# davipatti/abdpymc

Hardware: AMD Instinct MI355X
Metric: logp+grad evals/sec (higher is better)
Workload: dtype f64; 1 GPU; synthetic 10000 ind x 200 gaps, fp64, 4 chains/GPU; n_inds=10000, n_gaps=200, storage=f64, chains_per_gpu=4, total_chains=4, parallelism=chains sharded 4/GPU x 1

## Files before the change

### abdpymc_amd/csrc/abd_dense.hpp

```cpp
#pragma once

#include <cstddef>

#include "abd_device.hpp"
#include "abd_planes.hpp"
#include "abd_terms.hpp"

typedef uint32_t abd_u32x4 __attribute__((ext_vector_type(4)));
typedef uint32_t abd_u32x2 __attribute__((ext_vector_type(2)));
template <typename R>
__device__ __forceinline__ YX<R> load_yx(const __amdgpu_buffer_rsrc_t& rs, uint32_t voff, uint32_t soff);
template <>
__device__ __forceinline__ YX<double> load_yx<double>(const __amdgpu_buffer_rsrc_t& rs, uint32_t voff, uint32_t soff) {
  const abd_u32x4 v = __builtin_amdgcn_raw_buffer_load_b128(rs, voff, soff, 0);
  YX<double> r;
  r.y = __hiloint2double((int)v.y, (int)v.x);
  r.x = __hiloint2double((int)v.w, (int)v.z);
  return r;
}
template <>
__device__ __forceinline__ YX<float> load_yx<float>(const __amdgpu_buffer_rsrc_t& rs, uint32_t voff, uint32_t soff) {
  const abd_u32x2 v = __builtin_amdgcn_raw_buffer_load_b64(rs, voff, soff, 0);
  YX<float> r;
  r.y = __uint_as_float(v.x);
  r.x = __uint_as_float(v.y);
  return r;
}

template <typename R, bool XC>
struct RowData;
template <typename R>
struct RowData<R, false> {
  YX<R> v;
};
template <typename R>
struct RowData<R, true> {
  R y;
  uint32_t code;
};
template <bool XC>
struct RowDesc;
template <>
struct RowDesc<false> {
  __amdgpu_buffer_rsrc_t rs;
};
template <>
struct RowDesc<true> {
  __amdgpu_buffer_rsrc_t rs_y, rs_c;
};
__device__ __forceinline__ __amdgpu_buffer_rsrc_t rsrc_at(const void* base, int64_t byte_off) {
  return __builtin_amdgcn_make_buffer_rsrc(const_cast<char*>(reinterpret_cast<const char*>(base)) + byte_off, 0, -1, 0x00020000);
}
template <typename R, bool XC, typename ARGS>
__device__ __forceinline__ RowDesc<XC> row_desc(const ARGS& a, int antigen, int lg, int g0) {
  RowDesc<XC> d;
  if constexpr (XC) {
    const int64_t cell0 = ((int64_t)lg * a.G + g0) * 64;
    d.rs_y = rsrc_at(antigen ? a.od_s : a.od_n, cell0 * (int64_t)sizeof(R));
    d.rs_c = rsrc_at(antigen ? a.xc_s : a.xc_n, cell0);
  } else {
    const int64_t cell0 = (int64_t)g0 * a.N + (int64_t)lg * 64;
    d.rs = rsrc_at(antigen ? a.yx_s : a.yx_n, cell0 * (int64_t)sizeof(YX<R>));
  }
  return d;
}
template <typename R, bool XC>
__device__ __forceinline__ RowData<R, XC> row_load(const RowDesc<XC>& d, int lane, int row, int N) {
  RowData<R, XC> r;
  if constexpr (XC) {
    const uint32_t soff = (uint32_t)row * 64u;
    if constexpr (sizeof(R) == 8) {
      const abd_u32x2 v = __builtin_amdgcn_raw_buffer_load_b64(d.rs_y, (uint32_t)lane * 8u, soff * 8u, 0);
      r.y = __hiloint2double((int)v.y, (int)v.x);
    } else {
      r.y = __uint_as_float(__builtin_amdgcn_raw_buffer_load_b32(d.rs_y, (uint32_t)lane * 4u, soff * 4u, 0));
    }
    r.code = __builtin_amdgcn_raw_buffer_load_b8(d.rs_c, (uint32_t)lane, soff, 0);
  } else {
    r.v = load_yx<R>(d.rs, (uint32_t)lane * (uint32_t)sizeof(YX<R>), (uint32_t)row * (uint32_t)N * (uint32_t)sizeof(YX<R>));
  }
  return r;
}
template <typename R, bool XC>
__device__ __forceinline__ double row_y(const RowData<R, XC>& r) {
  if constexpr (XC) return (double)r.y;
  else return (double)r.v.y;
}
template <typename R, bool XC>
__device__ __forceinline__ double row_x(const RowData<R, XC>& r, const double* dict ) {
  if constexpr (XC) return dict[r.code];
  else return (double)r.v.x;
}

__device__ __forceinline__ uint32_t word32(const uint32_t* base, uint32_t j2, int q, int N) {
  const uint32_t* row = base + ((int64_t)(q >> 1) * 2 * N + (q & 1));
  return row[j2];
}

#define ABD_EXP2_C2 0x1.ebfbe033445b4p-23
__device__ __forceinline__ void one_plus_exp2_pair(double t_n, double t_s, const double* tab , double c2v, double& A,
                                                   double& B) {
#pragma clang fp contract(off)
  const double kf_n = __builtin_rint(t_n), kf_s = __builtin_rint(t_s);
  const double f_n = t_n - kf_n, f_s = t_s - kf_s;
  int k_n, k_s;
  asm("v_cvt_i32_f64 %0, %1" : "=v"(k_n) : "v"(kf_n));
  asm("v_cvt_i32_f64 %0, %1" : "=v"(k_s) : "v"(kf_s));
  const int kc_n = min(max(k_n, ABD_EXP2_K_MIN), ABD_EXP2_K_MAX), kc_s = min(max(k_s, ABD_EXP2_K_MIN), ABD_EXP2_K_MAX);
  const double T_n = tab[kc_n & (ABD_EXP2_TAB - 1)], T_s = tab[kc_s & (ABD_EXP2_TAB - 1)];
  double p_n, p_s;
  asm("v_fma_f64 %0, %1, %2, %3" : "=v"(p_n) : "s"(0x1.c6b08d910ecbdp-35), "v"(f_n), "v"(c2v));
  asm("v_fma_f64 %0, %1, %2, %3" : "=v"(p_s) : "s"(0x1.c6b08d910ecbdp-35), "v"(f_s), "v"(c2v));
  p_n = fma(p_n, f_n, 0x1.62e42fefa39efp-11);
  p_s = fma(p_s, f_s, 0x1.62e42fefa39efp-11);
  p_n = fma(p_n, f_n, 1.0);
  p_s = fma(p_s, f_s, 1.0);
  const double Ts_n = __hiloint2double((int)abd_exp2_scaled_hi((uint32_t)__double2hiint(T_n), kc_n), __double2loint(T_n));
  const double Ts_s = __hiloint2double((int)abd_exp2_scaled_hi((uint32_t)__double2hiint(T_s), kc_s), __double2loint(T_s));
  A = fma(Ts_n, p_n, 1.0);
  B = fma(Ts_s, p_s, 1.0);
}

template <bool GRAD>
__device__ __forceinline__ void obs_pair_scaled(double t_n, double yn, double d_n, double t_s, double ys, double d_s,
                                                const double* tab, double c2v, double (&acc)[16], double& h_n, double& h_s) {
#pragma clang fp contract(off)
  double A, B;
  one_plus_exp2_pair(t_n, t_s, tab, c2v, A, B);
  const double r = rcp_newton(A * B);
  const double s_n = r * B, s_s = r * A;
  const double q_n = fma(-d_n, s_n, yn), q_s = fma(-d_s, s_s, ys);
  acc[A_N_Q2] = fma(q_n, q_n, acc[A_N_Q2]);
  acc[A_S_Q2] = fma(q_s, q_s, acc[A_S_Q2]);
  if (GRAD) {
    const double u_n = q_n * s_n, u_s = q_s * s_s;
    acc[A_N_QS] = fma(s_n, q_n, acc[A_N_QS]);
    acc[A_S_QS] = fma(s_s, q_s, acc[A_S_QS]);
    h_n = fma(-u_n, s_n, u_n);
    h_s = fma(-u_s, s_s, u_s);
    acc[A_N_H] += h_n;
    acc[A_S_H] += h_s;
    acc[A_N_HX] = fma(h_n, t_n, acc[A_N_HX]);
    acc[A_S_HX] = fma(h_s, t_s, acc[A_S_HX]);
  }
}

#ifdef ABD_STAMPS
#define ABD_STAMP(k)                                                                                  \
  do {                                                                                                \
    if (a.stamps && wave == 0 && lane == 0 && blockIdx.y == 0)                                        \
      a.stamps[(int64_t)blockIdx.x * 16 + (k)] = __builtin_amdgcn_s_memrealtime();                   \
  } while (0)
#else
#define ABD_STAMP(k)
#endif

struct DenseChain {
  double rho_n, rho_s;
  double ct_n, cp_n, ci_n, mc_n;
  double c_s, cp_s, ci_s, mc_s;
  double d_n, d_s;
};
__device__ __forceinline__ DenseChain dense_chain(const ChainPar& p) {
  DenseChain k;
  const double c_n = p.b_n * (1.4426950408889634074 * ABD_EXP2_TAB), c_s = p.b_s * (1.4426950408889634074 * ABD_EXP2_TAB);
  k.rho_n = p.rho_n;
  k.rho_s = p.rho_s;
  k.ct_n = readfirstlane_f64(c_n * p.temp_n);
  k.cp_n = readfirstlane_f64(c_n * p.perm_n);
  k.ci_n = to_vgpr(c_n * p.init_n);
  k.mc_n = readfirstlane_f64(-c_n);
  k.c_s = readfirstlane_f64(c_s);
  k.cp_s = readfirstlane_f64(c_s * p.perm_s);
  k.ci_s = to_vgpr(c_s * p.init_s);
  k.mc_s = readfirstlane_f64(-c_s);
  k.d_n = p.d_n;
  k.d_s = p.d_s;
  return k;
}

#define ABD_SW 8
template <typename R, bool XC>
struct PieceLoads {
  uint32_t seg_i, seg_v, nxt_i, nxt_v;
  RowData<R, XC> en, es, on, os;
  int wj;
};

template <typename R, bool XC, bool WORDS, typename ARGS>
__device__ __forceinline__ void piece_issue_loads(const ARGS& a, const RowDesc<XC>& rs_n, const RowDesc<XC>& rs_s,
                                                  const uint32_t* ibase, const uint32_t* vbase, const int8_t* waner, int lane, int j,
                                                  int g0, int g1, PieceLoads<R, XC>& pl) {
  const int N = a.N;
  const int q = g0 >> 5, q_end = (g1 - 1) >> 5;
  const int last = g1 - 1 - g0;
  const int re = min(g0 & 1, last), ro = min((g0 & 1) ^ 1, last);
  if (g0 & 1) {
    pl.on = row_load<R, XC>(rs_n, lane, ro, N);
    pl.os = row_load<R, XC>(rs_s, lane, ro, N);
    pl.en = row_load<R, XC>(rs_n, lane, re, N);
    pl.es = row_load<R, XC>(rs_s, lane, re, N);
  } else {
    pl.en = row_load<R, XC>(rs_n, lane, re, N);
    pl.es = row_load<R, XC>(rs_s, lane, re, N);
    pl.on = row_load<R, XC>(rs_n, lane, ro, N);
    pl.os = row_load<R, XC>(rs_s, lane, ro, N);
  }
  pl.seg_i = pl.seg_v = pl.nxt_i = pl.nxt_v = 0;
  if constexpr (WORDS) {
    const uint32_t j2 = 2u * (uint32_t)j;
    pl.seg_i = word32(ibase, j2, q, N);
    pl.seg_v = word32(vbase, j2, q, N);
    if (q < q_end) {
      pl.nxt_i = word32(ibase, j2, q + 1, N);
      pl.nxt_v = word32(vbase, j2, q + 1, N);
    }
  }
  pl.wj = waner[j];
}

__device__ __forceinline__ void state_issue_loads(const uint32_t* ibase, const uint32_t* vbase, uint32_t j2, int N, int g0,
                                                  uint32_t (&wi)[ABD_SW], uint32_t (&wv)[ABD_SW]) {
  const int qlast = (g0 - 1) >> 5;
#pragma unroll
  for (int u = 0; u < ABD_SW; ++u) {
    wi[u] = wv[u] = 0;
    if (u <= qlast) {
      wi[u] = word32(ibase, j2, u, N);
      wv[u] = word32(vbase, j2, u, N);
    }
  }
}

__device__ __forceinline__ void dense_start_state(uint32_t (&wi)[ABD_SW], uint32_t (&wv)[ABD_SW], const uint32_t* ibase,
                                                  const uint32_t* vbase, uint32_t j2, int N, int g0, const double2_t* tab_n,
                                                  const double2_t* tab_s, bool wj, double& tn, double& dn, double& ts, double& ds,
                                                  uint32_t& cfn_hi, uint32_t& cfs_hi) {
  const int qlast = (g0 - 1) >> 5;
  uint32_t any_i = 0, any_v = 0;
  int cnt = 0;
  for (int q0 = 0;; q0 += ABD_SW) {
#pragma unroll
    for (int u = 0; u < ABD_SW; ++u) {
      const int q = q0 + u;
      if (q <= qlast) {
        const int rel = g0 - q * 32;
        uint32_t mi = wi[u], mv = wv[u];
        if (rel < 32) {
          const uint32_t below = (1u << rel) - 1u;
          mi &= below;
          mv &= below;
        }
        any_i |= mi;
        any_v |= mv;
        cnt += __builtin_popcount(mi) + __builtin_popcount(mv);
        if (__builtin_amdgcn_ballot_w64((mi | mv) != 0) != 0) {
          while (mi | mv) {
            const int idx_i = mi ? rel - __builtin_ctz(mi) : 0;
            const int idx_v = mv ? rel - __builtin_ctz(mv) : 0;
            mi &= mi - 1;
            mv &= mv - 1;
            const double2_t pn = tab_n[idx_i];
            const double2_t ps = tab_s[idx_i];
            const double2_t pv = tab_s[idx_v];
            tn += pn.x;
            dn += pn.y;
            ts += ps.x;
            ds += ps.y;
            ts += pv.x;
            ds += pv.y;
          }
        }
      }
    }
    if (q0 + ABD_SW > qlast) break;
#pragma unroll
    for (int u = 0; u < ABD_SW; ++u) {
      const int q = q0 + ABD_SW + u;
      wi[u] = wv[u] = 0;
      if (q <= qlast) {
        wi[u] = word32(ibase, j2, q, N);
        wv[u] = word32(vbase, j2, q, N);
      }
    }
  }
  if (!wj) {
    ts = (double)cnt;
    ds = 0.0;
  }
  cfn_hi = any_i ? 0x3FF00000u : 0u;
  cfs_hi = (any_i | any_v) ? 0x3FF00000u : 0u;
}

template <typename R, bool GRAD, bool XC, typename ARGS>
__device__ __forceinline__ void dense_walk(const ARGS& a, const DenseChain& k, const RowDesc<XC>& rs_n,
                                           const RowDesc<XC>& rs_s, const double* dict_n, const double* dict_s,
                                           const uint32_t* ibase, const uint32_t* vbase,
                                           uint32_t j2, PieceLoads<R, XC>& pl, int lane, int g0, int g1, bool wj, double tn, double dn, double ts,
                                           double ds, uint32_t cfn_hi, uint32_t cfs_hi, const double* tab_e2, double c2v,
                                           double (&acc)[16]) {
#pragma clang fp contract(off)
  const int N = a.N;
  const double rho_n = k.rho_n, ct_n = k.ct_n, cp_n = k.cp_n, ci_n = k.ci_n, mc_n = k.mc_n;
  const double c_s = k.c_s, cp_s = k.cp_s, ci_s = k.ci_s, mc_s = k.mc_s, d_n = k.d_n, d_s = k.d_s;
  const double rho_j = wj ? k.rho_s : 1.0;
  double hd_s = 0.0;
  const uint32_t z_ei = zero_vgpr(), z_ev = zero_vgpr(), z_cn = zero_vgpr(), z_cs = zero_vgpr();
  const int last = g1 - 1 - g0;
  auto ldrow = [&](const RowDesc<XC>& rs, int g) { return row_load<R, XC>(rs, lane, min(g - g0, last), N); };
  int q = g0 >> 5;
  const int q_end = (g1 - 1) >> 5;
  uint32_t seg_i = pl.seg_i, seg_v = pl.seg_v;
  auto next_word = [&]() {
    seg_i = pl.nxt_i;
    seg_v = pl.nxt_v;
    ++q;
    if (q < q_end) {
      pl.nxt_i = word32(ibase, j2, q + 1, N);
      pl.nxt_v = word32(vbase, j2, q + 1, N);
    }
  };

  auto step = [&](int g, const RowData<R, XC>& on, const RowData<R, XC>& os) {
    const uint32_t bit = (uint32_t)g & 31u;
    const uint32_t ei_hi = (uint32_t)__builtin_amdgcn_sbfe((int)seg_i, bit, 1u) & 0x3FF00000u;
    const uint32_t ev_hi = (uint32_t)__builtin_amdgcn_sbfe((int)seg_v, bit, 1u) & 0x3FF00000u;
    const double e_i = hi_to_double(ei_hi, z_ei), e_v = hi_to_double(ev_hi, z_ev);
    cfn_hi |= ei_hi;
    cfs_hi |= ei_hi | ev_hi;
    dn = fma_s(rho_n, dn, tn);
    tn = fma_s(rho_n, tn, e_i);
    ds = fma_v(rho_j, ds, ts);
    ts = fma_v(rho_j, ts, e_i + e_v);
    const double cf_n = hi_to_double(cfn_hi, z_cn), cf_s = hi_to_double(cfs_hi, z_cs);
    const double t_n = fma(mc_n, row_x<R, XC>(on, dict_n), fma(ct_n, tn, fma(cf_n, cp_n, ci_n)));
    const double t_s = fma(mc_s, row_x<R, XC>(os, dict_s), fma(c_s, ts, fma(cf_s, cp_s, ci_s)));
    double h_n = 0.0, h_s = 0.0;
    obs_pair_scaled<GRAD>(t_n, row_y<R, XC>(on), d_n, t_s, row_y<R, XC>(os), d_s, tab_e2, c2v, acc, h_n, h_s);
    if (GRAD) {
      acc[A_N_HC] = fma(h_n, cf_n, acc[A_N_HC]);
      acc[A_N_HU] = fma(h_n, tn, acc[A_N_HU]);
      acc[A_N_HD] = fma(h_n, dn, acc[A_N_HD]);
      acc[A_S_HC] = fma(h_s, cf_s, acc[A_S_HC]);
      hd_s = fma(h_s, ds, hd_s);
    }
  };

  RowData<R, XC> en = pl.en, es = pl.es, on = pl.on, os = pl.os;
  int g = g0;
  if (g & 1) {
    step(g, on, os);
    on = ldrow(rs_n, g + 2);
    os = ldrow(rs_s, g + 2);
    ++g;
    if (g < g1 && (g & 31) == 0) next_word();
  }
  while (g + 1 < g1) {
    const int pair_end = min(((g >> 5) + 1) << 5, g1 - 1);
    for (; g < pair_end; g += 2) {
      step(g, en, es);
      en = ldrow(rs_n, g + 2);
      es = ldrow(rs_s, g + 2);
      step(g + 1, on, os);
      on = ldrow(rs_n, g + 3);
      os = ldrow(rs_s, g + 3);
    }
    if (g < g1 && (g & 31) == 0) next_word();
  }
  if (g < g1) step(g, en, es);
  acc[A_S_HD] += wj ? hd_s : 0.0;
}


typedef uint64_t abd_u64x2 __attribute__((ext_vector_type(2)));
typedef uint64_t abd_u64x4 __attribute__((ext_vector_type(4)));
static_assert(sizeof(abd_u64x2) == sizeof(PlaneGap) && sizeof(abd_u64x4) == sizeof(PlanePair), "plane layout (abd_types.hpp)");
typedef const abd_u64x2 __attribute__((address_space(4)))* plane_gap_ptr;
typedef const abd_u64x4 __attribute__((address_space(4)))* plane_pair_ptr;
__device__ __forceinline__ plane_gap_ptr plane_row(const uint64_t* planes, int lg, int G) {
  return (plane_gap_ptr)(uintptr_t)(planes + abd_plane_index(lg, 0, G, 0));
}
__device__ __forceinline__ uint32_t mask_select(uint64_t mask, uint32_t on, uint32_t off) {
  return __builtin_amdgcn_inverse_ballot_w64(mask) ? on : off;
}

template <typename R, bool GRAD, bool XC, typename ARGS>
__device__ __forceinline__ void dense_walk_planes(const ARGS& a, const DenseChain& k, const RowDesc<XC>& rs_n,
                                                  const RowDesc<XC>& rs_s, const double* dict_n, const double* dict_s,
                                                  plane_gap_ptr prow, PieceLoads<R, XC>& pl, int lane, int g0, int g1, bool wj, double tn,
                                                  double dn, double ts, double ds, uint32_t cfn_hi, uint32_t cfs_hi, ExposureSeen seen,
                                                  const double* tab_e2, double c2v, double (&acc)[16]) {
#pragma clang fp contract(off)
  const int N = a.N;
  const double rho_n = k.rho_n, ct_n = k.ct_n, mc_n = k.mc_n;
  const double c_s = k.c_s, mc_s = k.mc_s, d_n = k.d_n, d_s = k.d_s;
  const double rho_j = wj ? k.rho_s : 1.0;
  double hd_s = 0.0;
  const uint32_t z_ei = zero_vgpr(), z_ev = zero_vgpr(), z_cn = zero_vgpr(), z_cs = zero_vgpr();
  const double b1_n = fma(1.0, k.cp_n, k.ci_n), b1_s = fma(1.0, k.cp_s, k.ci_s);
  double base_n = cfn_hi ? b1_n : fma(0.0, k.cp_n, k.ci_n), base_s = cfs_hi ? b1_s : fma(0.0, k.cp_s, k.ci_s);
  const int last = g1 - 1 - g0;
  auto ldrow = [&](const RowDesc<XC>& rs, int g) { return row_load<R, XC>(rs, lane, min(g - g0, last), N); };

  auto step = [&](uint64_t m_i, uint64_t m_v, const RowData<R, XC>& on, const RowData<R, XC>& os) {
    const ExposureSeen nw = abd_exposure_new(seen, m_i, m_v);
    if ((nw.n | nw.s) != 0) {
      cfn_hi = mask_select(nw.n, 0x3FF00000u, cfn_hi);
      cfs_hi = mask_select(nw.s, 0x3FF00000u, cfs_hi);
      base_n = __hiloint2double((int)mask_select(nw.n, (uint32_t)__double2hiint(b1_n), (uint32_t)__double2hiint(base_n)),
                                (int)mask_select(nw.n, (uint32_t)__double2loint(b1_n), (uint32_t)__double2loint(base_n)));
      base_s = __hiloint2double((int)mask_select(nw.s, (uint32_t)__double2hiint(b1_s), (uint32_t)__double2hiint(base_s)),
                                (int)mask_select(nw.s, (uint32_t)__double2loint(b1_s), (uint32_t)__double2loint(base_s)));
      abd_exposure_mark(seen, m_i, m_v);
    }
    const double e_i = hi_to_double(mask_select(m_i, 0x3FF00000u, 0u), z_ei), e_v = hi_to_double(mask_select(m_v, 0x3FF00000u, 0u), z_ev);
    dn = fma_s(rho_n, dn, tn);
    tn = fma_s(rho_n, tn, e_i);
    ds = fma_v(rho_j, ds, ts);
    ts = fma_v(rho_j, ts, e_i + e_v);
    const double cf_n = hi_to_double(cfn_hi, z_cn), cf_s = hi_to_double(cfs_hi, z_cs);
    const double t_n = fma(mc_n, row_x<R, XC>(on, dict_n), fma(ct_n, tn, base_n));
    const double t_s = fma(mc_s, row_x<R, XC>(os, dict_s), fma(c_s, ts, base_s));
    double h_n = 0.0, h_s = 0.0;
    obs_pair_scaled<GRAD>(t_n, row_y<R, XC>(on), d_n, t_s, row_y<R, XC>(os), d_s, tab_e2, c2v, acc, h_n, h_s);
    if (GRAD) {
      acc[A_N_HC] = fma(h_n, cf_n, acc[A_N_HC]);
      acc[A_N_HU] = fma(h_n, tn, acc[A_N_HU]);
      acc[A_N_HD] = fma(h_n, dn, acc[A_N_HD]);
      acc[A_S_HC] = fma(h_s, cf_s, acc[A_S_HC]);
      hd_s = fma(h_s, ds, hd_s);
      asm volatile("" : "+v"(cfn_hi), "+v"(cfs_hi), "+v"(base_n), "+v"(base_s), "+v"(acc[A_N_HC]), "+v"(acc[A_S_HC]));
    } else {
      asm volatile("" : "+v"(base_n), "+v"(base_s), "+v"(acc[A_N_Q2]), "+v"(acc[A_S_Q2]));
    }
  };

  RowData<R, XC> en = pl.en, es = pl.es, on = pl.on, os = pl.os;
  int g = g0;
  abd_u64x4 cur = *(plane_pair_ptr)(prow + ((g0 + 1) & ~1));
  if (g & 1) {
    const abd_u64x2 m = prow[g];
    step(m.x, m.y, on, os);
    on = ldrow(rs_n, g + 2);
    os = ldrow(rs_s, g + 2);
    ++g;
  }
  while (g + 1 < g1) {
    const abd_u64x4 nxt = *(plane_pair_ptr)(prow + g + 2);
    __builtin_amdgcn_sched_barrier(0);
    step(cur.x, cur.y, en, es);
    en = ldrow(rs_n, g + 2);
    es = ldrow(rs_s, g + 2);
    step(cur.z, cur.w, on, os);
    on = ldrow(rs_n, g + 3);
    os = ldrow(rs_s, g + 3);
    cur = nxt;
    g += 2;
  }
  if (g < g1) step(cur.x, cur.y, en, es);
  acc[A_S_HD] += wj ? hd_s : 0.0;
}

__device__ __forceinline__ const char* train_kernarg() {
#if defined(__HIP_DEVICE_COMPILE__)
  return (const char*)__builtin_amdgcn_kernarg_segment_ptr();
#else
  return nullptr;
#endif
}
__device__ __forceinline__ const TrainPoint* train_point(const TrainArgs& T) {
  return T.use_slot >= 0 ? T.slots + T.use_slot
                         : reinterpret_cast<const TrainPoint*>(train_kernarg() + offsetof(EvalArgs, train) + offsetof(TrainArgs, first));
}

__device__ __forceinline__ void train_forward_record(const TrainArgs& T, int lane) {
  const TrainPoint* cur = T.slots + T.use_slot;
  if (lane < ABD_NT) {
    T.fwd_rec->g[lane] = cur->prev_g[lane];
    T.fwd_rec->next_theta[lane] = cur->theta[lane];
    T.fwd_rec->next_p_half[lane] = cur->p_half[lane];
    if (lane == 0) T.fwd_rec->lp = cur->prev_lp;
  }
  __threadfence_system();
  __builtin_amdgcn_wave_barrier();
  if (lane == 0) __hip_atomic_store(&T.fwd_rec->tag, T.fwd_tag, __ATOMIC_RELEASE, __HIP_MEMORY_SCOPE_SYSTEM);
}

__device__ __forceinline__ void train_epilogue(const EvalArgs& a, double* sm, int lane) {
  const TrainArgs& T = a.train;
  const TrainPoint* cur = train_point(T);
  const double* inv_mass = reinterpret_cast<const double*>(train_kernarg() + offsetof(EvalArgs, train) + offsetof(TrainArgs, inv_mass));
  double* lps = sm + 16;
  const int k = lane < ABD_NT ? lane : 0;
  const int q4 = k == 0 ? 0 : k == 3 ? 1 : k == 6 ? 2 : k == 7 ? 3 : -1;
  abdi::Transformed tr;
  tr.p = cur->tr[0];
  tr.perm_n = cur->tr[1];
  tr.temp_n = cur->tr[2];
  tr.rho_n = cur->tr[3];
  tr.init_n = cur->tr[4];
  tr.perm_s = cur->tr[5];
  tr.rho_s = cur->tr[6];
  tr.q = cur->tr[7];
  tr.tinf = cur->tr[8];
  tr.tvac = cur->tr[9];
  tr.init_s = cur->tr[10];
  tr.b_n = cur->tr[11];
  tr.d_n = cur->tr[12];
  tr.sig_n = cur->tr[13];
  tr.b_s = cur->tr[14];
  tr.d_s = cur->tr[15];
  tr.sig_s = cur->tr[16];
  abdi::ModelSizes m;
  m.G = a.G;
  m.dense = 0;
  m.N = (double)a.N;
  m.cells = (double)a.G * (double)a.N;
  m.Kn = (double)a.K_n;
  m.Ks = (double)a.K_s;
  m.prior_const = T.prior_const;
  const double tk = cur->theta[k];
  const double l0 = q4 >= 0 ? cur->L0[q4] : 0.0, l1 = q4 >= 0 ? cur->L1[q4] : 0.0;
  double lp_k, g_k;
  abdi::assemble_lane(k, m, tr, tk, cur->tr[k], l0, l1, sm, lp_k, g_k);
  if (lane < ABD_NT) lps[lane] = lp_k;
  __builtin_amdgcn_wave_barrier();
  double lp = 0.0;
#pragma unroll
  for (int q = 0; q < ABD_NT; ++q) lp += lps[q];
  if (lane < ABD_NT) {
    if (T.own_record) {
      T.rec->g[lane] = g_k;
      if (lane == 0) T.rec->lp = lp;
    }
    const bool finite = __builtin_isfinite(lp);
    const double gd = finite ? g_k : 0.0;
    const double kick = __dmul_rn(__dmul_rn(0.5, T.ve), gd);
    const double p = __dadd_rn(cur->p_half[lane], kick);
    const double ph = __dadd_rn(p, kick);
    const double v = __dmul_rn(inv_mass[lane], ph);
    const double t2 = __dadd_rn(tk, __dmul_rn(T.ve, v));
    if (T.own_record) {
      T.rec->next_theta[lane] = t2;
      T.rec->next_p_half[lane] = ph;
    }
    double tr2, n0, n1;
    abdi::transform_lane(lane, t2, tr2, n0, n1);
    TrainPoint* nx = T.slots + T.next_slot;
    nx->theta[lane] = t2;
    nx->p_half[lane] = ph;
    nx->tr[lane] = tr2;
    if (q4 >= 0) {
      nx->L0[q4] = n0;
      nx->L1[q4] = n1;
    }
    nx->prev_g[lane] = g_k;
    if (lane == 0) nx->prev_lp = lp;
  }
  if (!T.own_record) return;
  __threadfence_system();
  __builtin_amdgcn_wave_barrier();
  if (lane == 0) __hip_atomic_store(&T.rec->tag, T.tag, __ATOMIC_RELEASE, __HIP_MEMORY_SCOPE_SYSTEM);
}

#define ABD_TRAIN_SM 64
__host__ __device__ inline size_t abd_dense_lds(int G, int cb, bool xc = false, bool train = false) {
  const size_t need = (size_t)cb * 2 * (size_t)(G + 1) * sizeof(double2_t) + (size_t)ABD_WAVES_PER_BLOCK * ABD_NOUT * sizeof(double) +
                      (size_t)ABD_EXP2_TAB * sizeof(double) + (xc ? (size_t)2 * ABD_XDICT * sizeof(double) : 0);
  const size_t fin = (size_t)ABD_FIN_PARTS * ABD_NOUT * sizeof(double) + (train ? (size_t)ABD_TRAIN_CB * ABD_TRAIN_SM * sizeof(double) : 0);
  return need > fin ? need : fin;
}

template <typename ARGS>
struct is_train_args {
  static constexpr bool value = false;
};
template <>
struct is_train_args<DenseTrainArgs> {
  static constexpr bool value = true;
};

__device__ __forceinline__ void train_service(const DenseTrainArgs& a, int wave, int lane);
__device__ __forceinline__ void train_step(const DenseTrainArgs& a, const TrainChainArgs& tc, double* sm, int lane);

template <int CB>
__device__ __forceinline__ bool two_level_sums(const double* rows, double* shard_rows, unsigned int* cnt, int nblk, int blk, unsigned int mask,
                                               int* flag, double* sm_chain, int tid) {
  const int lane = tid & 63, wave = tid >> 6;
  const int shard = blk % ABD_TRAIN_SHARDS;
  const int n_in_shard = (nblk - shard + ABD_TRAIN_SHARDS - 1) / ABD_TRAIN_SHARDS;
  const int n_shards = min(nblk, ABD_TRAIN_SHARDS);
  unsigned int* cnt_shard = cnt + (1 + shard) * ABD_TRAIN_CNT_STRIDE;
  if (wave == 0) {
    handoff_drain_stores();
    if (lane == 0) {
      const unsigned int old = handoff_count_in(cnt_shard);
      flag[0] = old + 1u == (unsigned int)n_in_shard ? 1 : 0;
    }
  }
  __syncthreads();
  const bool shard_last = flag[0] != 0;
  __syncthreads();
  if (!shard_last) return false;
  handoff_acquire();
  if (wave == 0) {
    if (lane < CB * ABD_NOUT) {
      const int cc = lane / ABD_NOUT, k = lane % ABD_NOUT;
      double v = 0.0;
      if ((mask >> cc) & 1u) {
        const double* col = rows + ((int64_t)cc * nblk + shard) * ABD_NOUT + k;
        for (int i0 = 0; i0 < n_in_shard; i0 += 8) {
          double q[8];
#pragma unroll
          for (int u = 0; u < 8; ++u)
            q[u] = i0 + u < n_in_shard ? __hip_atomic_load(col + (int64_t)(i0 + u) * ABD_TRAIN_SHARDS * ABD_NOUT, __ATOMIC_RELAXED, __HIP_MEMORY_SCOPE_AGENT) : 0.0;
#pragma unroll
          for (int u = 0; u < 8; ++u) v += q[u];
        }
      }
      __hip_atomic_store(shard_rows + ((int64_t)cc * ABD_TRAIN_SHARDS + shard) * ABD_NOUT + k, v, __ATOMIC_RELAXED, __HIP_MEMORY_SCOPE_AGENT);
    }
    handoff_drain_stores();
    if (lane == 0) {
      __hip_atomic_store(cnt_shard, 0u, __ATOMIC_RELAXED, __HIP_MEMORY_SCOPE_AGENT);
      const unsigned int old = handoff_count_in(cnt);
      flag[0] = old + 1u == (unsigned int)n_shards ? 1 : 0;
    }
  }
  __syncthreads();
  const bool last = flag[0] != 0;
  __syncthreads();
  if (!last) return false;
  handoff_acquire();
  if (wave == 0 && lane < CB * ABD_NOUT) {
    const int cc = lane / ABD_NOUT, k = lane % ABD_NOUT;
    const double* col = shard_rows + (int64_t)cc * ABD_TRAIN_SHARDS * ABD_NOUT + k;
    double v = 0.0;
    for (int i0 = 0; i0 < n_shards; i0 += 8) {
      double q[8];
#pragma unroll
      for (int u = 0; u < 8; ++u) q[u] = i0 + u < n_shards ? __hip_atomic_load(col + (int64_t)(i0 + u) * ABD_NOUT, __ATOMIC_RELAXED, __HIP_MEMORY_SCOPE_AGENT) : 0.0;
#pragma unroll
      for (int u = 0; u < 8; ++u) v += q[u];
    }
    sm_chain[cc * ABD_TRAIN_SM + k] = v;
  }
  if (tid == 0) __hip_atomic_store(cnt, 0u, __ATOMIC_RELAXED, __HIP_MEMORY_SCOPE_AGENT);
  __syncthreads();
  return true;
}

template <typename R, int CB, bool GRAD, bool XC, bool PL, typename ARGS>
__device__ __forceinline__ void dense_body(const ARGS& a) {
  constexpr bool TRAINK = is_train_args<ARGS>::value;
  static_assert(CB * ABD_NOUT <= 64, "the own-sum hand-off needs every partial row of the workgroup stored by wave 0");
  static_assert(!TRAINK || (GRAD && CB <= ABD_TRAIN_CB), "a train launch evaluates gradients for at most ABD_TRAIN_CB chains");
  extern __shared__ __align__(16) unsigned char smem[];
  const int G = a.G, N = a.N;
  const int tstride = G + 1;
  double2_t* tabs = reinterpret_cast<double2_t*>(smem);
  double* red = reinterpret_cast<double*>(tabs + CB * 2 * tstride);
  double* tab_e2 = red + ABD_WAVES_PER_BLOCK * ABD_NOUT;
  double* dict_n = tab_e2 + ABD_EXP2_TAB;
  double* dict_s = dict_n + ABD_XDICT;

  const int tid = threadIdx.x;
  const int lane = tid & 63;
  const int wave = __builtin_amdgcn_readfirstlane(tid >> 6);
  constexpr int NSUB = ABD_WAVES_PER_BLOCK / CB;
  const int c = wave % CB;
  const int sub = wave / CB;
  const int cbase = blockIdx.y * CB;
  int service = 0;
  if constexpr (TRAINK) {
    service = a.service;
    if (service && blockIdx.x == 0) {
      train_service(a, wave, lane);
      return;
    }
  }
  ChainPar p;
  bool chain_on = true;
  if constexpr (TRAINK) {
    const TrainChainArgs& tc = a.tc[c];
    chain_on = tc.action == ABD_TR_STEP;
    p.rw = nullptr;
    p.waner = tc.waner;
    p.iw = tc.iw;
    p.pl = tc.pl;
    p.cnt = tc.cnt;
    p.perm_n = p.temp_n = p.rho_n = p.init_n = p.perm_s = p.rho_s = p.init_s = p.b_n = p.d_n = p.b_s = p.d_s = 0.0;
    if (chain_on) {
      abdi::chain_par_from_tr(p, tc.st->pt[tc.use_slot].tr);
    }
  } else {
    p = a.ch[cbase + c];
  }

  ABD_STAMP(0);
  const int nblk = (int)gridDim.x - service;
  const int bid = (int)blockIdx.x - service;
  const int xcd = bid % 8, q8 = nblk / 8, rem8 = nblk % 8;
  const int blk = a.xcd_remap ? xcd * q8 + min(xcd, rem8) + bid / 8 : bid;

  if constexpr (!TRAINK) {
    const int n_fin = blockIdx.y == 0 ? a.prev_n_chains : 0;
    if (blk < n_fin) {
      finalize_chain<ABD_BLOCK>(a.prev_partials + (int64_t)blk * a.prev_blocks * ABD_NOUT, a.prev_blocks,
                     a.prev_out + (int64_t)blk * ABD_NOUT, reinterpret_cast<double*>(smem), tid, a.prev_tag);
      __syncthreads();
    }
  }

  double e2v[ABD_EXP2_TAB / ABD_BLOCK];
#pragma unroll
  for (int q = 0; q < ABD_EXP2_TAB / ABD_BLOCK; ++q) e2v[q] = a.exp2_tab[q * ABD_BLOCK + tid];
  double dv_n = 0.0, dv_s = 0.0;
  if (XC) {
    static_assert(ABD_XDICT == ABD_BLOCK, "one dictionary entry per thread");
    if (tid < a.n_dict_n) dv_n = a.dict_n[tid];
    if (tid < a.n_dict_s) dv_s = a.dict_s[tid];
  }

  auto range_start = [&](int r) { return r * a.rg_base + min(r, a.rg_extra) - a.rg_e_fin * min(r, a.rg_n_short); };
  auto range_of = [&](int r, int& r_lg, int& r_g0, int& r_rows) {
    const int pos = range_start(r);
    r_lg = G > 1 ? (int)__umulhi((uint32_t)pos, a.rg_g_magic) : pos;
    r_g0 = pos - r_lg * G;
    r_rows = range_start(r + 1) - pos;
  };
  int lg, g0, rows_left;
  range_of(blk * NSUB + sub, lg, g0, rows_left);
  if (TRAINK && !chain_on) rows_left = 0;
  int n_entries = rows_left > 0 ? g0 + 1 : 0;
#pragma unroll
  for (int s = 0; s < NSUB; ++s)
    if (NSUB > 1 && s != sub) {
      int o_lg, o_g0, o_rows;
      range_of(blk * NSUB + s, o_lg, o_g0, o_rows);
      n_entries = max(n_entries, o_rows > 0 ? o_g0 + 1 : 0);
    }
  if (TRAINK && !chain_on) n_entries = 0;
  ABD_STAMP(1);
#ifdef ABD_STAMPS
  if (a.stamps && wave == 0 && lane == 0 && blockIdx.y == 0) a.stamps[(int64_t)blockIdx.x * 16 + 9] = (unsigned long long)g0;
#endif

  const uint32_t* vbase = reinterpret_cast<const uint32_t*>(a.vw);
  const uint32_t* ibase = reinterpret_cast<const uint32_t*>(p.iw);
  PieceLoads<R, XC> pl;
  int g1 = min(G, g0 + rows_left);
  int j = lg * 64 + lane;
  uint32_t wi[ABD_SW], wv[ABD_SW];
  const bool first_inside = rows_left > 0 && j < N && g0 > 0;
  RowDesc<XC> rs_n = row_desc<R, XC>(a, 0, lg, g0), rs_s = row_desc<R, XC>(a, 1, lg, g0);
  if (rows_left > 0 && j < N) piece_issue_loads<R, XC, !PL>(a, rs_n, rs_s, ibase, vbase, p.waner, lane, j, g0, g1, pl);
  if (first_inside) state_issue_loads(ibase, vbase, 2u * (uint32_t)j, N, g0, wi, wv);
  long long n1 = 0, m1 = 0;
  if (blk == 0 && sub == 0 && chain_on) {
    n1 = p.cnt[0];
    m1 = p.cnt[1];
  }

  if (n_entries > 1) {
    if (NSUB >= 2) {
      if (sub == 0) fill_pow_table_wave(tabs + (c * 2 + 0) * tstride, p.rho_n, n_entries, lane);
      if (sub == 1) fill_pow_table_wave(tabs + (c * 2 + 1) * tstride, p.rho_s, n_entries, lane);
    } else {
      fill_pow_table_wave(tabs + (c * 2 + 0) * tstride, p.rho_n, n_entries, lane);
      fill_pow_table_wave(tabs + (c * 2 + 1) * tstride, p.rho_s, n_entries, lane);
    }
  }
  ABD_STAMP(2);
#pragma unroll
  for (int q = 0; q < ABD_EXP2_TAB / ABD_BLOCK; ++q) tab_e2[q * ABD_BLOCK + tid] = e2v[q];
  if (XC) {
    dict_n[tid] = dv_n;
    dict_s[tid] = dv_s;
  }
  ABD_STAMP(3);

  double acc[16];
#pragma unroll
  for (int k = 0; k < ABD_NACC; ++k) acc[k] = 0.0;

  const DenseChain kc = dense_chain(p);
  const double c2v = to_vgpr(ABD_EXP2_C2);
  const double2_t* tab_n = tabs + (c * 2 + 0) * tstride;
  const double2_t* tab_s = tabs + (c * 2 + 1) * tstride;
  if (NSUB == 1) {
    asm volatile("s_waitcnt lgkmcnt(0)" ::: "memory");
    __builtin_amdgcn_wave_barrier();
  } else {
    __syncthreads();
  }
  ABD_STAMP(4);

  double tn = 0.0, dn = 0.0, ts = 0.0, ds = 0.0;
  uint32_t cfn_hi = 0, cfs_hi = 0;
  ABD_STAMP(5);
  if (first_inside)
    dense_start_state(wi, wv, ibase, vbase, 2u * (uint32_t)j, N, g0, tab_n, tab_s, pl.wj != 0, tn, dn, ts, ds, cfn_hi, cfs_hi);
  ExposureSeen seen = {0, 0};
  if constexpr (PL) {
    seen.n = __builtin_amdgcn_ballot_w64(cfn_hi != 0);
    seen.s = __builtin_amdgcn_ballot_w64(cfs_hi != 0);
  }
  if (NSUB == 1) __syncthreads();
  ABD_STAMP(6);

  while (rows_left > 0) {
    rows_left -= g1 - g0;
    if (j < N) {
      if constexpr (PL)
        dense_walk_planes<R, GRAD, XC>(a, kc, rs_n, rs_s, dict_n, dict_s, plane_row(p.pl, lg, G), pl, lane, g0, g1, pl.wj != 0, tn, dn, ts, ds, cfn_hi,
                                       cfs_hi, seen, tab_e2, c2v, acc);
      else
        dense_walk<R, GRAD, XC>(a, kc, rs_n, rs_s, dict_n, dict_s, ibase, vbase, 2u * (uint32_t)j, pl, lane, g0, g1, pl.wj != 0, tn, dn, ts, ds, cfn_hi, cfs_hi,
                                tab_e2, c2v, acc);
    }
    if (rows_left <= 0) break;
    ++lg;
    g0 = 0;
    g1 = min(G, rows_left);
    j = lg * 64 + lane;
    tn = dn = ts = ds = 0.0;
    cfn_hi = cfs_hi = 0;
    seen.n = seen.s = 0;
    rs_n = row_desc<R, XC>(a, 0, lg, g0);
    rs_s = row_desc<R, XC>(a, 1, lg, g0);
    if (j < N) piece_issue_loads<R, XC, !PL>(a, rs_n, rs_s, ibase, vbase, p.waner, lane, j, g0, g1, pl);
  }

  ABD_STAMP(7);
  acc[ABD_NACC] = lane == 0 ? (double)n1 : 0.0;
  acc[ABD_NACC + 1] = lane == 0 ? (double)m1 : 0.0;
  acc[ABD_NACC + 2] = 0.0;
  const double tot = wave_reduce16(acc, lane);
  if ((lane & 3) == 0) red[wave * ABD_NOUT + reduce16_index(lane)] = tot;
  __syncthreads();
  bool own_sum = TRAINK;
  if constexpr (!TRAINK) own_sum = a.fin_count != nullptr;
  if (tid < CB * ABD_NOUT) {
    const int cc = tid / ABD_NOUT, k = tid % ABD_NOUT;
    double v = 0.0;
#pragma unroll
    for (int w = 0; w < NSUB; ++w) v += red[(w * CB + cc) * ABD_NOUT + k];
    double* dst = a.partials + ((int64_t)(cbase + cc) * nblk + blk) * ABD_NOUT + k;
    if (own_sum)
      __hip_atomic_store(dst, v, __ATOMIC_RELAXED, __HIP_MEMORY_SCOPE_AGENT);
    else
      *dst = v;
  }
  ABD_STAMP(8);
  if (!own_sum) return;

  int* flag = reinterpret_cast<int*>(red);
  __syncthreads();
  if constexpr (TRAINK) {
    if (nblk <= ABD_TRAIN_ONE_LEVEL) {
      if (wave == 0) {
        handoff_drain_stores();
        if (lane == 0) {
          const unsigned int old = handoff_count_in(a.fin_count);
          flag[0] = old + 1u == (unsigned int)nblk ? 1 : 0;
        }
      }
      __syncthreads();
      const bool last1 = flag[0] != 0;
      __syncthreads();
      if (!last1) return;
      ABD_STAMP(10);
      handoff_acquire();
      double* sm = reinterpret_cast<double*>(smem);
      double* sm_chain1 = sm + ABD_FIN_PARTS * ABD_NOUT;
#pragma unroll
      for (int cc = 0; cc < CB; ++cc) {
        if (a.tc[cc].action == ABD_TR_STEP) {
          sum_chain_coherent<ABD_BLOCK>(a.partials + (int64_t)cc * nblk * ABD_NOUT, nblk, sm, tid);
          if (tid < ABD_NOUT) sm_chain1[cc * ABD_TRAIN_SM + tid] = sm[tid];
          __syncthreads();
        }
      }
      ABD_STAMP(11);
      if (wave < CB && a.tc[wave].action != ABD_TR_SKIP) train_step(a, a.tc[wave], sm_chain1 + wave * ABD_TRAIN_SM, lane);
      ABD_STAMP(12);
      if (tid == 0) __hip_atomic_store(a.fin_count, 0u, __ATOMIC_RELAXED, __HIP_MEMORY_SCOPE_AGENT);
      return;
    }
    unsigned int step_mask = 0;
#pragma unroll
    for (int cc = 0; cc < CB; ++cc) step_mask |= a.tc[cc].action == ABD_TR_STEP ? 1u << cc : 0u;
    double* sm_chain = reinterpret_cast<double*>(smem);
    if (!two_level_sums<CB>(a.partials, a.partials + (int64_t)CB * nblk * ABD_NOUT, a.fin_count, nblk, blk, step_mask, flag, sm_chain, tid)) return;
    if (wave < CB && a.tc[wave].action != ABD_TR_SKIP) train_step(a, a.tc[wave], sm_chain + wave * ABD_TRAIN_SM, lane);
  } else if (a.fin_count != nullptr) {
    if (wave == 0) {
      handoff_drain_stores();
      if (lane < CB) {
        const unsigned int old = handoff_count_in(a.fin_count + cbase + lane);
        flag[lane] = old + 1u == gridDim.x ? 1 : 0;
      }
    }
    __syncthreads();
    bool last[CB];
#pragma unroll
    for (int cc = 0; cc < CB; ++cc) last[cc] = flag[cc] != 0;
    __syncthreads();
#pragma unroll
    for (int cc = 0; cc < CB; ++cc) {
      if (last[cc]) {
        handoff_acquire();
        finalize_chain_coherent<ABD_BLOCK>(a.partials + (int64_t)(cbase + cc) * gridDim.x * ABD_NOUT, (int)gridDim.x,
                                           a.fin_out + (int64_t)(cbase + cc) * ABD_NOUT, reinterpret_cast<double*>(smem), tid, a.fin_tag);
        if (tid == 0) __hip_atomic_store(a.fin_count + cbase + cc, 0u, __ATOMIC_RELAXED, __HIP_MEMORY_SCOPE_AGENT);
        __syncthreads();
      }
    }
  }
}

template <typename R, int CB, bool GRAD, bool XC, bool TRAIN>
struct dense_plane_form {
  static constexpr bool value = !TRAIN;
};

template <typename R, int CB, bool GRAD, bool XC, bool PL>
#ifndef ABD_DENSE_MINW
#define ABD_DENSE_MINW 4
#endif
__global__ __launch_bounds__(ABD_BLOCK, ABD_DENSE_MINW) void abd_dense_kernel(const EvalArgs a) {
  dense_body<R, CB, GRAD, XC, PL, EvalArgs>(a);
}

template <typename R, int CB, bool XC, bool PL>
__global__ __launch_bounds__(ABD_BLOCK, ABD_DENSE_MINW) void abd_train_kernel(const DenseTrainArgs a) {
  dense_body<R, CB, true, XC, PL, DenseTrainArgs>(a);
}
```

### abdpymc_amd/csrc/abd_planes.hpp

```cpp
#pragma once

#include "abd_types.hpp"

__host__ __device__ inline int abd_plane_gaps(int G) { return ((G + 1) & ~1) + 2; }
__host__ __device__ inline size_t abd_plane_words(int n_lg, int G) { return (size_t)n_lg * (size_t)abd_plane_gaps(G) * 2; }
__host__ __device__ inline size_t abd_plane_index(int lg, int g, int G, int which) {
  return ((size_t)lg * (size_t)abd_plane_gaps(G) + (size_t)g) * 2 + (size_t)which;
}

inline void abd_plane_transpose_ref(const uint64_t* words, int N, int G, int which, uint64_t* planes) {
  const int n_lg = (N + 63) / 64;
  for (int lg = 0; lg < n_lg; ++lg)
    for (int g = 0; g < G; ++g) {
      uint64_t m = 0;
      for (int l = 0; l < 64; ++l) {
        const int j = lg * 64 + l;
        if (j < N) m |= ((words[(size_t)(g >> 6) * N + j] >> (g & 63)) & 1ull) << l;
      }
      planes[abd_plane_index(lg, g, G, which)] = m;
    }
}

struct ExposureSeen {
  uint64_t n, s;
};
__host__ __device__ inline ExposureSeen abd_exposure_start(uint64_t infected_before, uint64_t vaccinated_before) {
  ExposureSeen s;
  s.n = infected_before;
  s.s = infected_before | vaccinated_before;
  return s;
}
__host__ __device__ inline ExposureSeen abd_exposure_new(const ExposureSeen& seen, uint64_t m_i, uint64_t m_v) {
  ExposureSeen nw;
  nw.n = m_i & ~seen.n;
  nw.s = (m_i | m_v) & ~seen.s;
  return nw;
}
__host__ __device__ inline void abd_exposure_mark(ExposureSeen& seen, uint64_t m_i, uint64_t m_v) {
  seen.n |= m_i;
  seen.s |= m_i | m_v;
}
```

Baseline: 256,800 evals/s.

## Compute exposure-gated gradient via running-sum differences instead of per-step FMA

Replaces the per-gap accumulation h*cf into the HC gradient accumulators with an open/close scheme: at the first exposure, subtract the running H sum, and at the end add it back, so HC equals the sum of h over gaps after first exposure. It also drops the cf_n/cf_s bit-to-double conversions and computes the serology boost e_i+e_v directly from plane masks as a single constant. This removes two FMAs plus conversions per step and frees registers in the inner loop. The trade-off is extra branching and ballot work on first-exposure events, and a different summation order (difference of partial sums), which changes the floating-point rounding.

```diff
diff --git a/abdpymc_amd/csrc/abd_dense.hpp b/abdpymc_amd/csrc/abd_dense.hpp
--- a/abdpymc_amd/csrc/abd_dense.hpp
+++ b/abdpymc_amd/csrc/abd_dense.hpp
@@ -292,7 +292,7 @@
   cfs_hi = (any_i | any_v) ? 0x3FF00000u : 0u;
 }
 
-template <typename R, bool GRAD, bool XC, typename ARGS>
+template <typename R, bool GRAD, bool XC, bool HCD, typename ARGS>
 __device__ __forceinline__ void dense_walk(const ARGS& a, const DenseChain& k, const RowDesc<XC>& rs_n,
                                            const RowDesc<XC>& rs_s, const double* dict_n, const double* dict_s,
                                            const uint32_t* ibase, const uint32_t* vbase,
@@ -306,6 +306,10 @@
   const double rho_j = wj ? k.rho_s : 1.0;
   double hd_s = 0.0;
   const uint32_t z_ei = zero_vgpr(), z_ev = zero_vgpr(), z_cn = zero_vgpr(), z_cs = zero_vgpr();
+  if constexpr (GRAD && HCD) {
+    acc[A_N_HC] = abd_hc_open(acc[A_N_HC], acc[A_N_H], cfn_hi != 0);
+    acc[A_S_HC] = abd_hc_open(acc[A_S_HC], acc[A_S_H], cfs_hi != 0);
+  }
   const int last = g1 - 1 - g0;
   auto ldrow = [&](const RowDesc<XC>& rs, int g) { return row_load<R, XC>(rs, lane, min(g - g0, last), N); };
   int q = g0 >> 5;
@@ -326,6 +330,13 @@
     const uint32_t ei_hi = (uint32_t)__builtin_amdgcn_sbfe((int)seg_i, bit, 1u) & 0x3FF00000u;
     const uint32_t ev_hi = (uint32_t)__builtin_amdgcn_sbfe((int)seg_v, bit, 1u) & 0x3FF00000u;
     const double e_i = hi_to_double(ei_hi, z_ei), e_v = hi_to_double(ev_hi, z_ev);
+    if constexpr (GRAD && HCD) {
+      const bool first_n = (ei_hi & ~cfn_hi) != 0, first_s = ((ei_hi | ev_hi) & ~cfs_hi) != 0;
+      if (__builtin_amdgcn_ballot_w64(first_n | first_s) != 0) {
+        acc[A_N_HC] = abd_hc_open(acc[A_N_HC], acc[A_N_H], first_n);
+        acc[A_S_HC] = abd_hc_open(acc[A_S_HC], acc[A_S_H], first_s);
+      }
+    }
     cfn_hi |= ei_hi;
     cfs_hi |= ei_hi | ev_hi;
     dn = fma_s(rho_n, dn, tn);
@@ -338,10 +349,10 @@
     double h_n = 0.0, h_s = 0.0;
     obs_pair_scaled<GRAD>(t_n, row_y<R, XC>(on), d_n, t_s, row_y<R, XC>(os), d_s, tab_e2, c2v, acc, h_n, h_s);
     if (GRAD) {
-      acc[A_N_HC] = fma(h_n, cf_n, acc[A_N_HC]);
+      if constexpr (!HCD) acc[A_N_HC] = fma(h_n, cf_n, acc[A_N_HC]);
       acc[A_N_HU] = fma(h_n, tn, acc[A_N_HU]);
       acc[A_N_HD] = fma(h_n, dn, acc[A_N_HD]);
-      acc[A_S_HC] = fma(h_s, cf_s, acc[A_S_HC]);
+      if constexpr (!HCD) acc[A_S_HC] = fma(h_s, cf_s, acc[A_S_HC]);
       hd_s = fma(h_s, ds, hd_s);
     }
   };
@@ -368,6 +379,10 @@
     if (g < g1 && (g & 31) == 0) next_word();
   }
   if (g < g1) step(g, en, es);
+  if constexpr (GRAD && HCD) {
+    acc[A_N_HC] = abd_hc_close(acc[A_N_HC], acc[A_N_H], cfn_hi != 0);
+    acc[A_S_HC] = abd_hc_close(acc[A_S_HC], acc[A_S_H], cfs_hi != 0);
+  }
   acc[A_S_HD] += wj ? hd_s : 0.0;
 }
 
@@ -388,48 +403,52 @@
 __device__ __forceinline__ void dense_walk_planes(const ARGS& a, const DenseChain& k, const RowDesc<XC>& rs_n,
                                                   const RowDesc<XC>& rs_s, const double* dict_n, const double* dict_s,
                                                   plane_gap_ptr prow, PieceLoads<R, XC>& pl, int lane, int g0, int g1, bool wj, double tn,
-                                                  double dn, double ts, double ds, uint32_t cfn_hi, uint32_t cfs_hi, ExposureSeen seen,
-                                                  const double* tab_e2, double c2v, double (&acc)[16]) {
+                                                  double dn, double ts, double ds, ExposureSeen seen, const double* tab_e2, double c2v,
+                                                  double (&acc)[16]) {
 #pragma clang fp contract(off)
   const int N = a.N;
   const double rho_n = k.rho_n, ct_n = k.ct_n, mc_n = k.mc_n;
   const double c_s = k.c_s, mc_s = k.mc_s, d_n = k.d_n, d_s = k.d_s;
   const double rho_j = wj ? k.rho_s : 1.0;
   double hd_s = 0.0;
-  const uint32_t z_ei = zero_vgpr(), z_ev = zero_vgpr(), z_cn = zero_vgpr(), z_cs = zero_vgpr();
+  const uint32_t z_ei = zero_vgpr(), z_eb = zero_vgpr();
   const double b1_n = fma(1.0, k.cp_n, k.ci_n), b1_s = fma(1.0, k.cp_s, k.ci_s);
-  double base_n = cfn_hi ? b1_n : fma(0.0, k.cp_n, k.ci_n), base_s = cfs_hi ? b1_s : fma(0.0, k.cp_s, k.ci_s);
+  const bool before_n = __builtin_amdgcn_inverse_ballot_w64(seen.n), before_s = __builtin_amdgcn_inverse_ballot_w64(seen.s);
+  double base_n = before_n ? b1_n : fma(0.0, k.cp_n, k.ci_n), base_s = before_s ? b1_s : fma(0.0, k.cp_s, k.ci_s);
+  if constexpr (GRAD) {
+    acc[A_N_HC] = abd_hc_open(acc[A_N_HC], acc[A_N_H], before_n);
+    acc[A_S_HC] = abd_hc_open(acc[A_S_HC], acc[A_S_H], before_s);
+  }
   const int last = g1 - 1 - g0;
   auto ldrow = [&](const RowDesc<XC>& rs, int g) { return row_load<R, XC>(rs, lane, min(g - g0, last), N); };
 
   auto step = [&](uint64_t m_i, uint64_t m_v, const RowData<R, XC>& on, const RowData<R, XC>& os) {
     const ExposureSeen nw = abd_exposure_new(seen, m_i, m_v);
     if ((nw.n | nw.s) != 0) {
-      cfn_hi = mask_select(nw.n, 0x3FF00000u, cfn_hi);
-      cfs_hi = mask_select(nw.s, 0x3FF00000u, cfs_hi);
+      if constexpr (GRAD) {
+        acc[A_N_HC] = abd_hc_open(acc[A_N_HC], acc[A_N_H], __builtin_amdgcn_inverse_ballot_w64(nw.n));
+        acc[A_S_HC] = abd_hc_open(acc[A_S_HC], acc[A_S_H], __builtin_amdgcn_inverse_ballot_w64(nw.s));
+      }
       base_n = __hiloint2double((int)mask_select(nw.n, (uint32_t)__double2hiint(b1_n), (uint32_t)__double2hiint(base_n)),
                                 (int)mask_select(nw.n, (uint32_t)__double2loint(b1_n), (uint32_t)__double2loint(base_n)));
       base_s = __hiloint2double((int)mask_select(nw.s, (uint32_t)__double2hiint(b1_s), (uint32_t)__double2hiint(base_s)),
                                 (int)mask_select(nw.s, (uint32_t)__double2loint(b1_s), (uint32_t)__double2loint(base_s)));
       abd_exposure_mark(seen, m_i, m_v);
     }
-    const double e_i = hi_to_double(mask_select(m_i, 0x3FF00000u, 0u), z_ei), e_v = hi_to_double(mask_select(m_v, 0x3FF00000u, 0u), z_ev);
+    const double e_i = hi_to_double(mask_select(m_i, 0x3FF00000u, 0u), z_ei);
+    const double e_b = hi_to_double(abd_s_boost_hi(__builtin_amdgcn_inverse_ballot_w64(m_i | m_v), __builtin_amdgcn_inverse_ballot_w64(m_i & m_v)), z_eb);
     dn = fma_s(rho_n, dn, tn);
     tn = fma_s(rho_n, tn, e_i);
     ds = fma_v(rho_j, ds, ts);
-    ts = fma_v(rho_j, ts, e_i + e_v);
-    const double cf_n = hi_to_double(cfn_hi, z_cn), cf_s = hi_to_double(cfs_hi, z_cs);
+    ts = fma_v(rho_j, ts, e_b);
     const double t_n = fma(mc_n, row_x<R, XC>(on, dict_n), fma(ct_n, tn, base_n));
     const double t_s = fma(mc_s, row_x<R, XC>(os, dict_s), fma(c_s, ts, base_s));
     double h_n = 0.0, h_s = 0.0;
     obs_pair_scaled<GRAD>(t_n, row_y<R, XC>(on), d_n, t_s, row_y<R, XC>(os), d_s, tab_e2, c2v, acc, h_n, h_s);
     if (GRAD) {
-      acc[A_N_HC] = fma(h_n, cf_n, acc[A_N_HC]);
       acc[A_N_HU] = fma(h_n, tn, acc[A_N_HU]);
       acc[A_N_HD] = fma(h_n, dn, acc[A_N_HD]);
-      acc[A_S_HC] = fma(h_s, cf_s, acc[A_S_HC]);
       hd_s = fma(h_s, ds, hd_s);
-      asm volatile("" : "+v"(cfn_hi), "+v"(cfs_hi), "+v"(base_n), "+v"(base_s), "+v"(acc[A_N_HC]), "+v"(acc[A_S_HC]));
     } else {
       asm volatile("" : "+v"(base_n), "+v"(base_s), "+v"(acc[A_N_Q2]), "+v"(acc[A_S_Q2]));
     }
@@ -458,6 +477,10 @@
     g += 2;
   }
   if (g < g1) step(cur.x, cur.y, en, es);
+  if constexpr (GRAD) {
+    acc[A_N_HC] = abd_hc_close(acc[A_N_HC], acc[A_N_H], __builtin_amdgcn_inverse_ballot_w64(seen.n));
+    acc[A_S_HC] = abd_hc_close(acc[A_S_HC], acc[A_S_H], __builtin_amdgcn_inverse_ballot_w64(seen.s));
+  }
   acc[A_S_HD] += wj ? hd_s : 0.0;
 }
 
@@ -813,10 +836,10 @@
     rows_left -= g1 - g0;
     if (j < N) {
       if constexpr (PL)
-        dense_walk_planes<R, GRAD, XC>(a, kc, rs_n, rs_s, dict_n, dict_s, plane_row(p.pl, lg, G), pl, lane, g0, g1, pl.wj != 0, tn, dn, ts, ds, cfn_hi,
-                                       cfs_hi, seen, tab_e2, c2v, acc);
+        dense_walk_planes<R, GRAD, XC>(a, kc, rs_n, rs_s, dict_n, dict_s, plane_row(p.pl, lg, G), pl, lane, g0, g1, pl.wj != 0, tn, dn, ts, ds, seen,
+                                       tab_e2, c2v, acc);
       else
-        dense_walk<R, GRAD, XC>(a, kc, rs_n, rs_s, dict_n, dict_s, ibase, vbase, 2u * (uint32_t)j, pl, lane, g0, g1, pl.wj != 0, tn, dn, ts, ds, cfn_hi, cfs_hi,
+        dense_walk<R, GRAD, XC, !TRAINK>(a, kc, rs_n, rs_s, dict_n, dict_s, ibase, vbase, 2u * (uint32_t)j, pl, lane, g0, g1, pl.wj != 0, tn, dn, ts, ds, cfn_hi, cfs_hi,
                                 tab_e2, c2v, acc);
     }
     if (rows_left <= 0) break;
diff --git a/abdpymc_amd/csrc/abd_planes.hpp b/abdpymc_amd/csrc/abd_planes.hpp
--- a/abdpymc_amd/csrc/abd_planes.hpp
+++ b/abdpymc_amd/csrc/abd_planes.hpp
@@ -40,3 +40,17 @@
   seen.n |= m_i;
   seen.s |= m_i | m_v;
 }
+
+__host__ __device__ inline double abd_hc_open(double hc, double H, bool lane_on) {
+  const double d = hc - H;
+  return lane_on ? d : hc;
+}
+__host__ __device__ inline double abd_hc_close(double hc, double H, bool lane_on) {
+  const double d = hc + H;
+  return lane_on ? d : hc;
+}
+
+__host__ __device__ inline uint32_t abd_s_boost_hi(bool either, bool both) {
+  const uint32_t one = either ? 0x3FF00000u : 0u;
+  return both ? 0x40000000u : one;
+}
```

Result: faster. 262,700 evals/s (median of 6 runs) (+2.3%).
